# rdevooght/sequence-based-recommendations

Hardware: AMD Instinct MI355X
Metric: user-sequences/sec training (ML-1M shape, seq200 b256) at 1/2/4/8 GPUs (higher is better)
Workload: dtype f32; 1 GPU; c2: train.py -m RNN --r_t GRU --r_l 128 --max_length 200 -b 256 --loss CCE --u_m adam, N=3706 items, Zipf(1.0) ids, lengths=full, 256 rows per GPU; global_batch=256, seq_len=200, parallelism=dp1

## Files before the change

### sequence-based-recommendations_amd/csrc/sbr_api.hip

```cpp
#include "sbr_common.h"
#include <stdarg.h>
#include <stdio.h>
#include <string.h>
#include <algorithm>
#include <stdlib.h>
#include <math.h>
#include <array>
#include <atomic>
#include <chrono>

static thread_local std::string g_err;
void sbr_set_error(const char* fmt, ...) {
    char buf[1024];
    va_list ap; va_start(ap, fmt); vsnprintf(buf, sizeof(buf), fmt, ap); va_end(ap);
    g_err = buf;
}
extern "C" const char* sbr_last_error(void) { return g_err.c_str(); }
extern "C" int sbr_abi_version(void) { return SBR_ABI_VERSION; }


int sbr_build_layout(const sbr_config& cfg, Layout& lay, std::string& err) {
    char buf[256];
#define LFAIL(...) do { snprintf(buf, sizeof(buf), __VA_ARGS__); err = buf; return SBR_EINVAL; } while (0)
    if (cfg.abi_version != SBR_ABI_VERSION) LFAIL("abi_version %d != %d", cfg.abi_version, SBR_ABI_VERSION);
// ... 739 lines not shown
}

__global__ void __launch_bounds__(256) occupy_kernel(unsigned long long ticks, int* sink) {
    extern __shared__ int occ_lds[];
    occ_lds[threadIdx.x] = (int)threadIdx.x;
    const unsigned long long t0 = wall_clock64();
    while (wall_clock64() - t0 < ticks) __builtin_amdgcn_s_sleep(64);
    if (occ_lds[(threadIdx.x + 1) & 255] == -7) *sink = 1;
}
extern "C" int sbr_debug_occupy(sbr_handle* h, int workgroups, int lds_kb, int milliseconds) {
    CHECK_ARG(h && workgroups >= 0 && workgroups <= 4096 && lds_kb >= 0 && lds_kb <= 160 && milliseconds >= 0 && milliseconds <= 10000, "bad argument");
    static hipStream_t occ = nullptr;
    if (!occ) SBR_HIP(hipStreamCreateWithFlags(&occ, hipStreamNonBlocking));
    if (workgroups == 0) { SBR_HIP(hipStreamSynchronize(occ)); return SBR_OK; }
    const size_t lds = std::max<size_t>(1024, (size_t)lds_kb * 1024);
    SBR_DYN_LDS(occupy_kernel, lds);
    occupy_kernel<<<workgroups, 256, lds, occ>>>((unsigned long long)milliseconds * 100000ull, (int*)h->A(h->lay.a_fault) + 1);
    SBR_LAUNCH(hipGetLastError());
    return SBR_OK;
}

extern "C" int sbr_query(sbr_handle* h, const char* what, int64_t* value) {
    CHECK_ARG(h && what && value, "null argument");
    const Layout& y = h->lay; const std::string w(what);
    const RecPlan& top = h->plan[(y.L - 1) * y.D];
    if (w == "fused_gather") *value = h->plan[0].fuse_gather ? 1 : 0;
    else if (w == "rows_per_workgroup") *value = h->rpt;
    else if (w == "head_fused") {
        int cc = 0, cw = 0; size_t lds = 0;
        *value = (h->sw.head_fuse && y.cfg.loss == SBR_LOSS_CCE && !simple_gemm(h) && !(y.cfg.flags & (SBR_FLAG_BF16_PROJECTION | SBR_FLAG_F32_MFMA)) &&
                  y.D == 1 && y.B == y.Bp && sbr_head_plan(y.Bp, y.N, y.HLt, &cc, &cw, &lds) && (size_t)cc * y.Bp * y.HLt <= y.ws_floats) ? cc : 0;
    }
    else if (w == "head_sampled") *value = head_sampled_taken(h, y.B) ? 1 : 0;
    else if (w == "scatter_form") *value = h->last_scatter_form;
    else if (w == "step_join_gate") *value = h->last_join_gate;
    else if (w == "step_fork_gate") *value = h->last_fork_gate;
    else if (w == "tail_gate_first") *value = h->last_tail_gated;
    else if (w == "rank_select") *value = h->last_rank_select;
    else if (w == "rank_sort") *value = h->last_rank_sort;
    else if (w == "cluster_rank_form") *value = h->last_cluster_rank_form;
    else if (w == "goal_rank_form") *value = h->last_goal_rank_form;
    else if (w == "goal_rank_tile") *value = kGoalRankTile;
    else if (w == "row_aware_update") *value = h->last_row_aware ? 1 : 0;
    else if (w == "cluster") *value = top.needs_fill ? 1 : 0;
    else if (w == "rec_kernel") *value = top.family;
    else if (w.rfind("rec_products_", 0) == 0 || w.rfind("rec_rows_", 0) == 0 || w.rfind("rec_workgroups_", 0) == 0) {
        const bool bwd = w.size() > 4 && w.compare(w.size() - 4, 4, "_bwd") == 0;
        *value = w.rfind("rec_products_", 0) == 0 ? (bwd ? top.products_bwd : top.products_fwd)
               : w.rfind("rec_rows_", 0) == 0 ? (bwd ? top.bwd_rows : top.fwd_rows) : (bwd ? top.bwd_wgs : top.fwd_wgs);
    }
    else if (w == "tail_chunks") *value = h->tail_chunks;
    else if (w == "tail_streams") *value = (h->tail_chunks >= 2 && h->sw.tail_overlap == 1) ? 1 : 0;
    else if (w == "tail_last_steps") *value = h->tail_chunks >= 2 ? h->tail_bounds.lo[1] : 0;
    else if (w == "side_stream2") *value = (int64_t)(intptr_t)h->side2;
    else if (w == "tail_chain_cycles" || w == "tail_chain_ticks") {
        unsigned long long c[2] = {0, 0};
        const int nwaves = (y.Bp / h->rpt) * 8;
        SBR_HIP(hipStreamSynchronize(h->stream));
        SBR_HIP(hipMemcpy(c, (const int*)h->A(y.a_prog) + nwaves + 128, sizeof(c), hipMemcpyDeviceToHost));
        *value = (int64_t)c[w == "tail_chain_cycles" ? 0 : 1];
    }
    else if (w == "tail_win_lo") *value = (int64_t)y.layer[0].p_Win;
    else if (w == "tail_win_hi") *value = (int64_t)y.layer[0].p_b;
    else if (w == "tail_whid_lo") *value = (int64_t)y.layer[0].p_Whid;
    else if (w == "tail_whid_hi") *value = (int64_t)y.layer[0].p_peep;
    else if (w == "arena_bytes") *value = (int64_t)(y.s_end * sizeof(float));
    else if (w == "sparse_blocks") *value = y.n_sparse;
    else if (w == "adam_table") *value = y.n_at;
    else if (w == "side_stream") *value = (int64_t)(intptr_t)h->side;
    else { sbr_set_error("unknown query '%s'", what); return SBR_EINVAL; }
    return SBR_OK;
}

extern "C" int sbr_enable_timing(sbr_handle* h, int on) {
    CHECK_ARG(h, "null handle");
    if (on)
        for (int r = 0; r < sbr_handle::kRing; ++r)
            for (int i = 0; i < SBR_N_PHASES; ++i) if (!h->ev[r][i]) SBR_HIP(hipEventCreate(&h->ev[r][i]));
    CHECK_ARG(on >= 0 && on <= SBR_N_PHASES, "on = %d: 0 off, 1 every phase, 2 + p only phase p", on);
    h->timing = on != 0; h->ring_used = 0; h->ring_cur = 0;
    h->timing_marks = on == 1 ? 0xffu : on >= 2 ? (3u << (on - 2)) : 0u;
    return SBR_OK;
}

extern "C" int sbr_chain_times(sbr_handle* h, int on, float us[2], int n[2]) {
    CHECK_ARG(h, "null handle");
    if (on) { h->ch_n = 0; h->chain_timing = true; return SBR_OK; }
    CHECK_ARG(us && n, "null argument");
    h->chain_timing = false;
    SBR_HIP(hipDeviceSynchronize());
    us[0] = us[1] = 0.f; n[0] = n[1] = 0;
    for (int r = 0; r < h->ch_n; ++r) {
        float ms = 0.f;
        if (!h->ev_ch[r][0] || !h->ev_ch[r][1] || hipEventElapsedTime(&ms, h->ev_ch[r][0], h->ev_ch[r][1]) != hipSuccess) continue;
        us[h->ch_dir[r] & 1] += ms * 1000.f; n[h->ch_dir[r] & 1] += 1;
    }
    h->ch_n = 0;
    return SBR_OK;
}

extern "C" int sbr_phase_times(sbr_handle* h, float us[SBR_N_PHASES]) {
    CHECK_ARG(h && us, "null argument");
    if (!h->timing || h->ring_used == 0) { sbr_set_error("no timed train step recorded"); return SBR_ESTATE; }
    SBR_HIP(hipStreamSynchronize(h->stream));
    const int n = std::min(h->ring_used, (int)sbr_handle::kRing);
    for (int i = 0; i < SBR_N_PHASES; ++i) us[i] = 0.f;
// ... 11 lines not shown
```

### sequence-based-recommendations_amd/csrc/sbr_common.h

```cpp
#pragma once
#include <hip/hip_runtime.h>
#include <stdint.h>
#include <stddef.h>
#include <math.h>
#include <string>
#include <vector>
#include "../../include/sbr_rnn.h"
#include "sbr_upd.h"

#define SBR_BWD_CHUNKS 4
#define SBR_ALIGN_FLOATS 64

static inline size_t sbr_align(size_t n_floats) { return (n_floats + SBR_ALIGN_FLOATS - 1) / SBR_ALIGN_FLOATS * SBR_ALIGN_FLOATS; }
static inline int sbr_gates(int cell) { return cell == SBR_CELL_LSTM ? 4 : (cell == SBR_CELL_GRU ? 3 : 1); }
static inline int sbr_pad_hidden(int H) {
    if (H <= 16) return 16;
    if (H <= 32) return 32;
    if (H <= 64) return 64;
    if (H <= 128) return 128;
    if (H <= 256) return 256;
    if (H <= 512) return 512;
    return (H + 63) / 64 * 64;
}

// ... 50 lines not shown
    size_t a_dhl[2];
    size_t a_dinp[2];
    size_t a_s2cnt, a_s2off, a_s2cur, a_s2sid, a_s2pos;
    int E, Ep;
    size_t p_Emb;
    size_t a_emb, a_demb;
    LayerLayout layer[2 * SBR_MAX_LAYERS];
    size_t p_WoutT, p_bout;
    size_t n_params;
    size_t p_split;
    size_t n_state_arrays;
    size_t s_params, s_grads, s_state, s_act, s_end;
    size_t a_logits;
    size_t a_dhlast;
    size_t a_rowcost;
    int NT;
    size_t a_dflt;
    size_t a_Wc, a_bc, a_act, a_dWc, a_dbc;
    size_t a_ws; size_t ws_floats;
    size_t a_ws2; size_t ws2_floats;
    size_t a_csum;
    size_t a_prof;
    size_t a_fault;
    size_t a_clx;
    size_t a_X, a_len, a_tgt, a_smp, a_cells, a_pop, a_topk;
    size_t a_X2, a_len2, a_tgt2, a_smp2, a_pop2;
    size_t a_scnt, a_soff, a_scur, a_sid, a_spos;
    size_t a_sP;
    size_t a_hstat;
    size_t a_srpart, a_srid; int sr_slots;
    int tail_keys;
    size_t a_prog;
    size_t a_done;
};

int sbr_build_layout(const sbr_config& cfg, Layout& lay, std::string& err);

struct ParamDesc { std::string name; int layer; int kind; int gate; int64_t d0, d1; int ndim; };
void sbr_param_descs(const Layout& lay, std::vector<ParamDesc>& out);

#define SBR_TCHUNKS_MAX 9
struct SbrTChunks { int n; int lo[SBR_TCHUNKS_MAX + 1]; };
constexpr int kWgradSlices = 256;
constexpr int kWgradX6Wgs = 512;
constexpr int kTailChunksMax = 8;
constexpr int kTailPubEvery = 2;
constexpr int kTailShortChunks = 3;
constexpr int kTailFenceKb = 124;
constexpr int kTailFirst = 6;
constexpr int kTailScatterUnits = 192;
constexpr int kTailGemmGroups = 64;
constexpr int kTailSlabMax = 512;
constexpr double kTailSlabGrowth = 0.35;
constexpr bool kTailGateFirst = true;
constexpr int kTailGateSleep = 32;
constexpr bool kStepJoinGate = true;
constexpr bool kStepForkGate = true;
static inline double sbr_tail_geom(int scatter_lds) { return scatter_lds ? 1.6 : 2.6; }

enum ScatForm { SCAT_REDUCE = 0, SCAT_RANGE = 1, SCAT_WIDE = 2, SCAT_ATOMIC = 3, SCAT_POLL = 4, SCAT_LDS = 5 };
struct ScatReduce { int nv; bool comb; };
struct ScatPlan {
    ScatForm plain = SCAT_REDUCE, tail = SCAT_POLL;
    ScatReduce reduce = {0, false};
    int range_nv = 0, wide_nvw = 0, wide_nvb = 0;
    int poll_nv = 0;
    int lds_nv = 0, floor_cost = 0, rows_lds = 0;
    bool wide_rows = false;
};
static inline bool sbr_scatter_wide_rows(int Ep, int GHp) { return !Ep && GHp >= 512 && GHp <= 8192; }
static inline int sbr_scatter_wide_slots(size_t max_entries) { return (int)(max_entries / 64 + max_entries / 65 + 2); }
ScatReduce sbr_scat_reduce_recipe(int row_floats);
ScatPlan sbr_scat_plan(int GHp, int Ep, int n_ids, int entries, int D, bool atomic, int scat_range, int tail_scatter_lds,
                       int tail_chunks, int units, int part_slots);
constexpr int kRankThreads = 1024;
constexpr int kRankLdsRow = 32768;
constexpr int kRankSortLds = 2048;
constexpr int kGoalRankTile = 1024;
static_assert(kGoalRankTile == kRankThreads, "ev_goal_rank_kernel: a thread owns one goal item of the tile and one word of its scan");

__device__ __forceinline__ unsigned rank_key(float v) {
    if (!(v > -INFINITY)) return 0u;
    unsigned u = __float_as_uint(v);
    if (v == 0.0f) u = 0u;
    return (u & 0x80000000u) ? ~u : (u | 0x80000000u);
}

struct UserSplit {
    int L, half, fed;
    __host__ __device__ constexpr UserSplit(long long off_lo, long long off_hi, int T)
        : L((int)(off_hi - off_lo)), half(L / 2), fed(T < half ? T : half) {}
    __host__ __device__ constexpr int goal_len() const { return L - half; }
    __host__ __device__ constexpr int viewed_begin() const { return 0; }
    __host__ __device__ constexpr int viewed_end() const { return half; }
    __host__ __device__ constexpr int window_begin() const { return half - fed; }
    __host__ __device__ constexpr int window_end() const { return half; }
};
#define SBR_SPLIT_IS(L, T, H, G, WB) (UserSplit(100, 100 + (L), (T)).half == (H) && UserSplit(100, 100 + (L), (T)).goal_len() == (G) && \
                                      UserSplit(100, 100 + (L), (T)).window_begin() == (WB) && UserSplit(100, 100 + (L), (T)).window_end() == (H))
static_assert(SBR_SPLIT_IS(2, 0, 1, 1, 1) && SBR_SPLIT_IS(2, 1, 1, 1, 0) && SBR_SPLIT_IS(2, 5, 1, 1, 0), "L = 2: one item viewed, one the goal");
static_assert(SBR_SPLIT_IS(3, 0, 1, 2, 1) && SBR_SPLIT_IS(3, 1, 1, 2, 0) && SBR_SPLIT_IS(3, 2, 1, 2, 0), "L = 3: the odd item belongs to the goal");
static_assert(SBR_SPLIT_IS(7, 2, 3, 4, 1) && SBR_SPLIT_IS(7, 3, 3, 4, 0) && SBR_SPLIT_IS(7, 4, 3, 4, 0), "L = 7: the window is the END of the viewed half");
#undef SBR_SPLIT_IS

#define HEAD_WAIT_TICKS 6000ull
struct SbrSwitches {
// ... 168 lines not shown
void plan_tail(sbr_handle* h);
bool head_sampled_taken(const sbr_handle* h, int rows);
void mark(sbr_handle* h, int i);
SbrSparseRows sparse_rows(sbr_handle* h, int b);
SbrSparseUpd sparse_upd(sbr_handle* h);
int side_join(sbr_handle* h);
static inline bool sparse_lazy(const sbr_handle* h) { return h->lay.n_sparse > 0 && h->lay.cfg.updater != SBR_UPD_ADAGRAD; }
struct SbrSortKeys { int *cnt, *off, *cur, *sid, *pos; };
SbrSortKeys sort_keys(const sbr_handle* h, int dir);
std::vector<std::pair<size_t, size_t>> sparse_float_ranges(const Layout& lay);

#define SBR_DYN_LDS(KERNEL, LDS) do { static int sbr_dyn_lds_set_ = -1; if ((int)(LDS) > sbr_dyn_lds_set_) { \
        (void)hipFuncSetAttribute((const void*)KERNEL, hipFuncAttributeMaxDynamicSharedMemorySize, (int)(LDS)); sbr_dyn_lds_set_ = (int)(LDS); } } while (0)
#define SBR_DONE_COPIES 32
#define SBR_DONE_STRIDE 1088
struct SbrPoll { const int* words; int n; int* done; int epoch; int rows_per_step; int* fault; int n_small, k_small;
                 unsigned long long* trace; const int* slab_lo; int n_slabs; };

hipError_t launch_gather_xt(hipStream_t s, const float* Win, const float* bias, const int* X, float* xt,
                            int T, int Bp, int F, int GHp, int n_rows_in);
hipError_t launch_scatter_rows(hipStream_t s, float* dWin, const float* dxt, const int* X, const int* len,
                               int T, int Bp, int F, int GHp);
hipError_t launch_scatter_sort(hipStream_t s, const int* X, const int* len, int T, int Bp, int F, int n_ids, int* cnt,
                               int* offs, int* cur, int* sid, int* spos, int concat = 0, int tch = 0, int n_tchunks = 1, const SbrTChunks* bounds = nullptr,
                               int* cnt_zero_n = nullptr);
int sbr_scatter_lds_ids();
hipError_t launch_tail_gate(hipStream_t s, const int* progress, int n, int epoch, int target, int* fault);
hipError_t launch_tail_gate_wave(hipStream_t s, const int* progress, int n, int epoch, int target, int* fault);
hipError_t launch_step_gate(hipStream_t s, const int* w0, const int* w1, int epoch, int* fault);
hipError_t launch_step_word(hipStream_t s, int* word, int epoch);
hipError_t launch_gather_concat(hipStream_t s, const float* Wemb, const int* X, float* out, int T, int Bp, int F, int Ep);
hipError_t launch_rev_rows_int(hipStream_t s, const int* X, const int* len, int* Xr, int T, int Bp, int F);
hipError_t launch_rev_rows(hipStream_t s, const float* src, const int* len, float* dst, int T, int Bp, int W);
hipError_t launch_cat_outputs(hipStream_t s, const float* hs_f, const float* hs_b, const int* len, float* cat, int T, int Bp, int Hp);
hipError_t launch_hcat(hipStream_t s, const float* hf, const float* hb, float* out, int Bp, int Hp);
hipError_t launch_split_cols(hipStream_t s, const float* src, float* a, float* b, int rows, int Hp);
hipError_t launch_uncat(hipStream_t s, const float* f, const float* r, const int* len, float* out_f, float* out_b, int T, int Bp,
                        int W, int Hp);
hipError_t launch_scatter_range(hipStream_t s, float* dWin, const float* dxt, const int* sid, const int* spos, const int* offs, int n_ids,
                                int GHp, float* part, int* part_id, int n_ranges, const ScatPlan& plan);
#define SBR_SCAT_RANGES 512
hipError_t launch_scatter_wide(hipStream_t s, float* dWin, const float* dxt, const int* sid, const int* spos, const int* offs, int n_ids,
                               int max_entries, int GHp, float* part, int* aux, int n_slots, const ScatPlan& plan);
hipError_t launch_scatter_reduce(hipStream_t s, float* dWin, const float* dxt, const int* sid, const int* spos,
                                 const int* offs, int n_ids, int max_entries, int GHp, int Bp, const ScatReduce& recipe);
hipError_t launch_scatter_reduce_poll(hipStream_t s, float* dWin, const float* dxt, const int* sid, const int* spos, const int* offs,
                                      int n_ids, int n_tchunks, int max_entries, int GHp, int Bp, const SbrPoll& poll,
                                      const SbrTChunks& bounds, int short_chunks, bool fence_on, const ScatPlan& plan);
hipError_t launch_scatter_cost_scan(hipStream_t s, const int* offs, int* P, int n_ids, int n_tchunks, const ScatPlan& plan);
hipError_t launch_scatter_lds_poll(hipStream_t s, float* dWin, const float* dxt, const int* sid, const int* spos, const int* offs, const int* P,
                                   int n_ids, int n_tchunks, int GHp, const SbrPoll& poll, const SbrTChunks& bounds,
                                   int units, const ScatPlan& plan, bool monitor = false, int t_lo = 0);
hipError_t launch_tail_monitor(hipStream_t s, const SbrPoll& poll, int t_lo);

__host__ __device__ __forceinline__ size_t sbr_blocked_index(int t, int row, int col, int Bp, int ncols) {
    return (((size_t)t * (Bp >> 4) + (row >> 4)) * (ncols >> 4) + (col >> 4)) * 256 + (row & 15) * 16 + (col & 15);
}

struct RecArgs {
    int cell, T, Bp, H, Hp, G;
    float clip;
    const int* len;
    const float* xt;
    const float* Whid;
    const float* peep;
    const float* cinit;
    const float* hinit;
    float* hs; float* cs; float* g[4];
    const float* dh_last;
    const float* dh_slabs;
    int n_dh_slabs;
    const float* dh_ext;
    int dhe_on;
    float* dxt; float* dhi;
    int t_lo, t_hi, chunk;
    float* state;
    float* part;
    int rpt;
    int xt_blocked;
    int x6_pipe;
    int x6_f16, x6_f16_bwd;
    int cl16, c16_two_level;
    const int* gX;
    const float* gWin;
    int n_in;
    const float* gbias;
    int f32_mfma;
    unsigned long long* prof;
    int cluster;
    int cl_linear;
    int* fault;
    int sentinel_done;
    int* clx;
    void* xh;
    float* pring;
    int epoch;
    int relu;
    int* progress; int prog_every; int prog_epoch;
    int* start_word; int start_epoch;
    int fence_kb;
};
static inline bool sbr_rec_f16_fwd(const RecArgs& a) { return a.x6_f16 && !a.relu; }
static inline bool sbr_rec_f16_bwd(const RecArgs& a) { return a.x6_f16_bwd && a.clip > 0.0f && a.clip <= 100.0f; }
#define SBR_CL_ROWS 8
#define SBR_C16_RING 2
#define SBR_X6P_FUSE_MAX_T 4096
// ... 128 lines not shown
```

### sequence-based-recommendations_amd/csrc/sbr_misc.hip

```cpp
#include "sbr_common.h"
#include "sbr_rec_p.h"
#include "sbr_device.h"
#include <math.h>

typedef float f32x4 __attribute__((ext_vector_type(4)));


__global__ void gather_xt_kernel(const f32x4* __restrict__ Win, const f32x4* __restrict__ bias,
                                 const int* __restrict__ X, f32x4* __restrict__ xt, int T, int Bp, int F, int R4) {
    const size_t total = (size_t)T * Bp * R4;
    for (size_t i = (size_t)blockIdx.x * blockDim.x + threadIdx.x; i < total; i += (size_t)gridDim.x * blockDim.x) {
        const int f4 = (int)(i % R4);
        const size_t pos = i / R4;
        const int b = (int)(pos % Bp), t = (int)(pos / Bp);
        f32x4 v = bias[f4];
        const int* ids = X + ((size_t)b * T + t) * F;
        for (int f = 0; f < F; ++f) v += Win[(size_t)ids[f] * R4 + f4];
        xt[i] = v;
    }
}

__global__ void gather_concat_kernel(const f32x4* __restrict__ W, const int* __restrict__ X, f32x4* __restrict__ out, int T,
                                     int Bp, int F, int E4) {
    const size_t total = (size_t)T * Bp * F * E4;
// ... 76 lines not shown
    const int w = i % (2 * Hp), r = i / (2 * Hp);
    if (w < Hp) a[(size_t)r * Hp + w] = src[i]; else b[(size_t)r * Hp + w - Hp] = src[i];
}
hipError_t launch_split_cols(hipStream_t s, const float* src, float* a, float* b, int rows, int Hp) {
    split_cols_kernel<<<(rows * 2 * Hp + 255) / 256, 256, 0, s>>>(src, a, b, rows, Hp);
    return hipGetLastError();
}

__global__ void uncat_kernel(const float* __restrict__ f, const float* __restrict__ r, const int* __restrict__ len,
                             float* __restrict__ out_f, float* __restrict__ out_b, int T, int Bp, int W, int Hp) {
    const size_t total = (size_t)T * Bp * W;
    for (size_t i = (size_t)blockIdx.x * blockDim.x + threadIdx.x; i < total; i += (size_t)gridDim.x * blockDim.x) {
        const int w = (int)(i % W);
        const size_t pos = i / W;
        const int b = (int)(pos % Bp), t = (int)(pos / Bp);
        const int tr = rev_t(t, len[b]);
        const float d = f[i] + r[((size_t)tr * Bp + b) * W + w];
        if (!out_b) out_f[i] = d;
        else if (w < Hp) out_f[((size_t)t * Bp + b) * Hp + w] = d;
        else out_b[((size_t)tr * Bp + b) * Hp + (w - Hp)] = d;
    }
}
hipError_t launch_uncat(hipStream_t s, const float* f, const float* r, const int* len, float* out_f, float* out_b, int T, int Bp,
                        int W, int Hp) {
    const size_t total = (size_t)T * Bp * W;
    uncat_kernel<<<(int)min((size_t)4096, (total + 255) / 256), 256, 0, s>>>(f, r, len, out_f, out_b, T, Bp, W, Hp);
    return hipGetLastError();
}

hipError_t launch_gather_xt(hipStream_t s, const float* Win, const float* bias, const int* X, float* xt, int T, int Bp,
                            int F, int GHp, int) {
    const int R4 = GHp / 4;
    const size_t total = (size_t)T * Bp * R4;
    const int grid = (int)min((size_t)256 * 16, (total + 255) / 256);
    gather_xt_kernel<<<grid, 256, 0, s>>>((const f32x4*)Win, (const f32x4*)bias, X, (f32x4*)xt, T, Bp, F, R4);
    return hipGetLastError();
}

__global__ void __launch_bounds__(512) tail_gate_kernel(const int* __restrict__ progress, int n, int epoch, int target, int* __restrict__ fault) {
    for (int i = threadIdx.x; i < n; i += blockDim.x) {
        const unsigned long long t0 = wall_clock64();
        for (;;) {
            const int v = __hip_atomic_load(progress + i, __ATOMIC_RELAXED, __HIP_MEMORY_SCOPE_AGENT);
            if ((v >> 12) == epoch && (v & 0xfff) <= target) break;
            if (wall_clock64() - t0 > SBR_POLL_TICKS) { atomicOr(fault, 8); break; }
            __builtin_amdgcn_s_sleep(8);
        }
    }
}

__global__ void __launch_bounds__(256) tail_monitor_kernel(SbrPoll pl, int t_lo) { tail_monitor_loop(pl, t_lo); }
hipError_t launch_tail_monitor(hipStream_t s, const SbrPoll& poll, int t_lo) {
    tail_monitor_kernel<<<1, 256, 0, s>>>(poll, t_lo);
    return hipGetLastError();
}

hipError_t launch_tail_gate(hipStream_t s, const int* progress, int n, int epoch, int target, int* fault) {
    tail_gate_kernel<<<1, 512, 0, s>>>(progress, n, epoch, target, fault);
    return hipGetLastError();
}

__global__ void __launch_bounds__(64) tail_gate_wave_kernel(const int* __restrict__ progress, int n, int epoch, int target, int* __restrict__ fault) {
    const unsigned long long t0 = wall_clock64();
    auto passed = [&](int v) { return (v >> 12) == epoch && (v & 0xfff) <= target; };
    for (;;) {
        if (passed(__hip_atomic_load(progress, __ATOMIC_RELAXED, __HIP_MEMORY_SCOPE_AGENT))) break;
        if (wall_clock64() - t0 > SBR_POLL_TICKS) { if (threadIdx.x == 0) atomicOr(fault, 8); return; }
        __builtin_amdgcn_s_sleep(kTailGateSleep);
    }
    for (;;) {
        bool ok = true;
#pragma unroll 8
        for (int i = 0; i < n; i += 64)
            ok = passed(__hip_atomic_load(progress + min(i + (int)threadIdx.x, n - 1), __ATOMIC_RELAXED, __HIP_MEMORY_SCOPE_AGENT)) && ok;
        if (__all(ok)) break;
        if (wall_clock64() - t0 > SBR_POLL_TICKS) { if (threadIdx.x == 0) atomicOr(fault, 8); return; }
        __builtin_amdgcn_s_sleep(8);
    }
}
hipError_t launch_tail_gate_wave(hipStream_t s, const int* progress, int n, int epoch, int target, int* fault) {
    if (n < 1) return hipErrorInvalidValue;
    tail_gate_wave_kernel<<<1, 64, 0, s>>>(progress, n, epoch, target, fault);
    return hipGetLastError();
}

__global__ void __launch_bounds__(64) step_gate_kernel(const int* __restrict__ w0, const int* __restrict__ w1, int epoch, int* __restrict__ fault) {
    const unsigned long long t0 = wall_clock64();
    for (;;) {
        const int a = __hip_atomic_load(w0, __ATOMIC_RELAXED, __HIP_MEMORY_SCOPE_AGENT);
        const int b = w1 ? __hip_atomic_load(w1, __ATOMIC_RELAXED, __HIP_MEMORY_SCOPE_AGENT) : epoch;
        if (a == epoch && b == epoch) break;
        if (wall_clock64() - t0 > SBR_POLL_TICKS) { if (threadIdx.x == 0) atomicOr(fault, 8); return; }
        __builtin_amdgcn_s_sleep(8);
    }
}
hipError_t launch_step_gate(hipStream_t s, const int* w0, const int* w1, int epoch, int* fault) {
    if (!w0 || !epoch) return hipErrorInvalidValue;
    step_gate_kernel<<<1, 64, 0, s>>>(w0, w1, epoch, fault);
    return hipGetLastError();
}
__global__ void __launch_bounds__(64) step_word_kernel(int* __restrict__ word, int epoch) {
    if (threadIdx.x == 0) __hip_atomic_store(word, epoch, __ATOMIC_RELAXED, __HIP_MEMORY_SCOPE_AGENT);
}
hipError_t launch_step_word(hipStream_t s, int* word, int epoch) {
    if (!word || !epoch) return hipErrorInvalidValue;
    step_word_kernel<<<1, 64, 0, s>>>(word, epoch);
// ... 335 lines not shown
```

### sequence-based-recommendations_amd/csrc/sbr_scatter.hip

```cpp
#include "sbr_common.h"
#include "sbr_rec_p.h"

#define SCAT_LDS_IDS 36864
#define SCAT_BLOCK 1024
__device__ __forceinline__ int scat_key(int id, int t, const SbrTChunks& tc, int ids_per_chunk) {
    if (tc.n <= 1) return id;
    int c = 0;
#pragma unroll
    for (int k = 1; k < SBR_TCHUNKS_MAX; ++k) c += (k < tc.n && t >= tc.lo[k]) ? 1 : 0;
    return c * ids_per_chunk + id;
}

__global__ void __launch_bounds__(SCAT_BLOCK) scat_count_lds_kernel(const int* __restrict__ X, const int* __restrict__ len,
                                                                    int T, int Bp, int F, int n_ids, int per_block,
                                                                    int* __restrict__ cnt, SbrTChunks tch, int ipc) {
    extern __shared__ int hist[];
    for (int i = threadIdx.x; i < n_ids; i += SCAT_BLOCK) hist[i] = 0;
    __syncthreads();
    const int total = T * Bp * F;
    const int lo = blockIdx.x * per_block, hi = min(total, lo + per_block);
    for (int i = lo + threadIdx.x; i < hi; i += SCAT_BLOCK) {
        const int f = i % F, pos = i / F, b = pos % Bp, t = pos / Bp;
        if (t < len[b]) atomicAdd(&hist[scat_key(X[((size_t)b * T + t) * F + f], t, tch, ipc)], 1);
    }
// ... 166 lines not shown
        const int f = i % F; pos = i / F;
        const int b = pos % Bp, t = pos / Bp;
        if (t < len[b]) { id = X[((size_t)b * T + t) * F + f]; h = scat_agg_insert(hkey, hcnt, id, rank); }
    }
    __syncthreads();
    for (int k = threadIdx.x; k < SCAT_AGG_SLOTS; k += 1024) if (hkey[k] >= 0) hbase[k] = atomicAdd(&cur[hkey[k]], hcnt[k]);
    __syncthreads();
    if (id >= 0) { const int slot = hbase[h] + rank; sid[slot] = id; spos[slot] = concat ? i : pos; }
}

int sbr_scatter_lds_ids() { return SCAT_LDS_IDS; }

hipError_t launch_scatter_sort(hipStream_t s, const int* X, const int* len, int T, int Bp, int F, int n_ids, int* cnt,
                               int* offs, int* cur, int* sid, int* spos, int concat, int tch, int n_tchunks, const SbrTChunks* bounds,
                               int* cnt_zero_n) {
    const int ipc = n_ids;
    const SbrTChunks tc = bounds ? *bounds : SbrTChunks{};
    if (tch > 0) {
        n_ids *= n_tchunks;
        if (n_ids > SCAT_LDS_IDS || tc.n != n_tchunks || tc.n > SBR_TCHUNKS_MAX || tc.lo[0] != 0 || tc.lo[tc.n] < T) return hipErrorInvalidValue;
    }
    if (!(cnt_zero_n && *cnt_zero_n >= n_ids)) {
        hipError_t e = hipMemsetAsync(cnt, 0, (size_t)n_ids * sizeof(int), s);
        if (e != hipSuccess) return e;
    }
    if (cnt_zero_n) *cnt_zero_n = n_ids <= SCAT_LDS_IDS ? n_ids : 0;
    const int total = T * Bp * F;
    if (n_ids <= SCAT_LDS_IDS) {
        const int per_block = 4096;
        const int grid = (total + per_block - 1) / per_block;
        const size_t lds = (size_t)n_ids * sizeof(int);
        SBR_DYN_LDS(scat_count_lds_kernel, lds);
        SBR_DYN_LDS(scat_fill_lds_kernel, lds);
        scat_count_lds_kernel<<<grid, SCAT_BLOCK, lds, s>>>(X, len, T, Bp, F, n_ids, per_block, cnt, tc, ipc);
        SBR_DYN_LDS(scat_scan_kernel<true>, lds);
        scat_scan_kernel<true><<<1, 1024, lds, s>>>(cnt, n_ids, offs, cur);
        scat_fill_lds_kernel<<<grid, SCAT_BLOCK, lds, s>>>(X, len, T, Bp, F, n_ids, per_block, cur, sid, spos, concat, tc, ipc);
    } else {
        const int agrid = (total + 1023) / 1024;
        scat_count_agg_kernel<<<agrid, 1024, 0, s>>>(X, len, T, Bp, F, cnt);
        const int nb = (n_ids + SCAN_BLK - 1) / SCAN_BLK;
        if (nb <= 1) scat_scan_kernel<false><<<1, 1024, 0, s>>>(cnt, n_ids, offs, cur);
        else {
            scat_scan_local_kernel<<<nb, 1024, 0, s>>>(cnt, n_ids, offs, cur);
            scat_scan_totals_kernel<<<1, 1024, 0, s>>>(cur, nb, cnt, offs + n_ids);
            scat_scan_add_kernel<<<nb, 1024, 0, s>>>(cnt, n_ids, offs, cur);
        }
        scat_fill_agg_kernel<<<agrid, 1024, 0, s>>>(X, len, T, Bp, F, cur, sid, spos, concat);
    }
    return hipGetLastError();
}

#define SCAT_FLY 8
template <int NV, int SCAT_CHUNK, bool ACC = false, bool POLL = false>
__global__ void __launch_bounds__(256) scat_reduce_kernel(const f32x4* __restrict__ dxt, const int* __restrict__ sid,
                                                          const int* __restrict__ spos, const int* __restrict__ offs,
                                                          int n_ids, float* __restrict__ dWin, int R4, int Bp, int key_lo = 0,
                                                          int n_tchunks = 1, SbrTChunks tch = SbrTChunks(), SbrPoll poll = SbrPoll()) {
    constexpr int FLY = (NV == 1 && !POLL) ? 16 : SCAT_FLY;
    const int lane = threadIdx.x & 63;
    const int wave_global = blockIdx.x * (blockDim.x >> 6) + (threadIdx.x >> 6), n_waves = gridDim.x * (blockDim.x >> 6);
    const int total = offs[POLL ? n_ids * n_tchunks : key_lo + n_ids];
    const int e_lo = POLL ? offs[key_lo] : 0;
    constexpr int SCAT_SHORT = 8;
    const int e_mid = POLL ? max(e_lo, min(total, offs[min(poll.n_small, n_tchunks) * n_ids])) : 0;
    const int nchA = POLL ? (total - e_mid + SCAT_CHUNK - 1) / SCAT_CHUNK : 0, nchB = POLL ? (e_mid - e_lo + SCAT_SHORT - 1) / SCAT_SHORT : 0;
    for (int it = wave_global; ; it += n_waves) {
    int base, cnt;
    if (POLL) {
        if (it >= nchA + nchB) break;
        if (it < nchA) { base = e_mid + (nchA - 1 - it) * SCAT_CHUNK; cnt = min(SCAT_CHUNK, total - base); }
        else { base = e_lo + (nchB - 1 - (it - nchA)) * SCAT_SHORT; cnt = min(SCAT_SHORT, e_mid - base); }
    } else {
        base = offs[key_lo] + wave_global * SCAT_CHUNK;
        if (base >= total) return;
        cnt = min(SCAT_CHUNK, total - base);
    }
    const int lim = base + cnt;
    const int e = base + (lane & (SCAT_CHUNK - 1));
    const int my_id = e < lim ? sid[e] : -1;
    const int my_pos = e < lim ? spos[e] : 0;
    if (POLL) {
        const int t_need = tch.lo[min(__shfl(my_id, 0) / n_ids, SBR_TCHUNKS_MAX)];
        if (lane == 0) {
            const unsigned long long t0 = wall_clock64();
            const int* mine = poll.done + ((blockIdx.x + 16) & (SBR_DONE_COPIES - 1)) * SBR_DONE_STRIDE;
            for (;;) {
                const int v = __hip_atomic_load(mine, __ATOMIC_RELAXED, __HIP_MEMORY_SCOPE_AGENT);
                if ((v >> 12) == poll.epoch && (v & 0xfff) <= t_need) break;
                if (wall_clock64() - t0 > SBR_POLL_TICKS) { atomicOr(poll.fault, 8); break; }
                poll_sleep((v >> 12) == poll.epoch ? (v & 0xfff) - t_need : 64);
            }
        }
        __builtin_amdgcn_wave_barrier();
        if (poll.trace && lane == 0) {
            const int k = min((it - wave_global) / n_waves, 3);
            poll.trace[8192 + (wave_global * 4 + k) * 2] = wall_clock64();
        }
    }
    f32x4 acc[NV];
#pragma unroll
    for (int v = 0; v < NV; ++v) acc[v] = f32x4{0, 0, 0, 0};
    int cur_id = __shfl(my_id, 0);
#ifndef SCAT_DEBUG_NOFLUSH
#define SCAT_DEBUG_NOFLUSH 0
#endif
// ... 654 lines not shown
```

### sequence-based-recommendations_amd/csrc/sbr_step.hip

```cpp
#include "sbr_common.h"
#include <string.h>
#include <algorithm>
#include <atomic>
#include <chrono>

static inline unsigned long long* prof_slot(const sbr_handle* h, int k) {
    return (unsigned long long*)h->A(h->lay.a_prof) + (size_t)k * (h->lay.Bp / 16) * 16 * 8;
}
static RecArgs rec_shape(const sbr_handle* h, int l) {
    const Layout& y = h->lay; const LayerLayout& ly = y.layer[l];
    RecArgs a; memset(&a, 0, sizeof(a));
    a.cell = y.cfg.cell; a.T = y.T; a.Bp = y.Bp; a.H = ly.H; a.Hp = ly.Hp; a.G = y.G;
    a.n_in = ly.n_in_p;
    a.clip = y.cfg.grad_clip;
    a.rpt = h->rpt; a.x6_pipe = h->sw.x6_pipe; a.x6_f16 = h->sw.x6_f16; a.x6_f16_bwd = h->sw.x6_f16_bwd;
    a.cl16 = h->sw.cl16; a.c16_two_level = h->sw.c16_two_level;
    a.hs = h->A(ly.a_hs); a.cs = h->A(ly.a_cs);
    for (int k = 0; k < 4; ++k) a.g[k] = h->A(ly.a_g[k]);
    if (ly.Hp == 256 || ly.Hp == 512) { a.xh = h->A(ly.a_xh); a.pring = h->A(ly.a_pring); }
    a.f32_mfma = (y.cfg.flags & SBR_FLAG_F32_MFMA) ? 1 : 0;
    a.prof = (y.cfg.flags & SBR_FLAG_PROFILE_REC) ? prof_slot(h, 0) : nullptr;
    a.cluster = h->sw.cluster; a.cl_linear = h->sw.cl_linear;
    a.relu = (y.cfg.cell == SBR_CELL_VANILLA && (l / y.D > 0 || y.E)) ? 1 : 0;
    return a;
// ... 1 lines not shown
static RecArgs rec_args(sbr_handle* h, int l) {
    const Layout& y = h->lay; const LayerLayout& ly = y.layer[l];
    RecArgs a = rec_shape(h, l);
    a.len = h->blen;
    a.xt = h->A(ly.a_xt); a.Whid = h->P(ly.p_Whid); a.peep = h->P(ly.p_peep);
    a.cinit = h->P(ly.p_cinit); a.hinit = h->P(ly.p_hinit);
    a.dxt = h->A(ly.a_dxt); a.dhi = h->A(ly.a_dhi); a.part = h->A(ly.a_part);
    a.xt_blocked = 0;
    a.t_lo = 0; a.t_hi = y.T; a.chunk = 0; a.state = h->A(ly.a_state);
    a.fault = (int*)h->A(y.a_fault);
    a.clx = (int*)h->A(y.a_clx); a.epoch = (++h->cl_epoch) & 0x07FFFFFF;
    return a;
}
static bool simple_rec(const sbr_handle* h) { return h->lay.cfg.flags & SBR_FLAG_SIMPLE_REC; }
void plan_layers(sbr_handle* h) {
    const Layout& y = h->lay;
    for (int l = 0; l < y.L * y.D; ++l) {
        RecArgs a = rec_shape(h, l);
        if (l / y.D < y.L - 1) a.dh_ext = h->A(y.layer[l].a_dhext);
        h->plan[l] = sbr_rec_plan(a, simple_rec(h), l / y.D == 0 && !y.E && y.F == 1 && h->sw.fuse_gather);
    }
}
static const RecPlan& plan_of(const sbr_handle* h, const LayerLayout& ly) { return h->plan[&ly - h->lay.layer]; }
static inline bool layer_gemm_f16(const sbr_handle* h, bool with_gradient) {
    const Layout& y = h->lay;
    if (!h->sw.gemm_f16 || y.cfg.cell == SBR_CELL_VANILLA) return false;
    return !with_gradient || (y.cfg.grad_clip > 0.0f && y.cfg.grad_clip <= 100.0f);
}
static inline void layer_gemm_hint(const sbr_handle* h, bool grad_a, bool grad_b) {
    if (h->lay.cfg.flags & SBR_FLAG_BF16_LAYERS) sbr_gemm_hint(1, 1.0f, 1.0f);
    else if (layer_gemm_f16(h, grad_a || grad_b)) sbr_gemm_hint(2, grad_a ? 512.0f : 1.0f, grad_b ? 512.0f : 1.0f);
}
bool simple_gemm(const sbr_handle* h) { return h->lay.cfg.flags & SBR_FLAG_SIMPLE_GEMM; }
bool head_sampled_taken(const sbr_handle* h, int rows) {
    const Layout& y = h->lay;
    return h->sw.head_fuse && !simple_gemm(h) && y.D == 1 && !(y.cfg.flags & SBR_FLAG_F32_MFMA) &&
           sbr_head_sampled_ok(rows, y.C, y.HLt, y.cfg.loss);
}
void plan_tail(sbr_handle* h) {
    const Layout& y = h->lay;
    h->tail_chunks = h->tail_ch = 0;
    if (!h->sw.tail_overlap || y.tail_keys < 2 || y.n_sparse || h->sw.bwd_chunks != 1) return;
    if (!h->plan[0].tail_ok || simple_gemm(h) || (y.cfg.flags & SBR_FLAG_ATOMIC_SCATTER)) return;
    int nc = std::min(std::min(y.tail_keys, kTailChunksMax), y.T / 16);
    if (nc < 2) return;
    const int ch = (y.T + nc - 1) / nc;
    nc = (y.T + ch - 1) / ch;
    if (nc < 2) return;
    h->tail_chunks = nc; h->tail_ch = ch;
    const double geom = sbr_tail_geom(h->sw.tail_scatter_lds);
    SbrTChunks& tc = h->tail_bounds;
    tc.n = nc;
    tc.lo[0] = 0;
    double pw = h->sw.tail_scatter_lds ? (double)kTailFirst : 1.0;
    for (int c = 0; c < nc; ++c) {
        const int rem = y.T - tc.lo[c], left = nc - c;
        const int share = (rem + left - 1) / left;
        const int n_small = nc >= 4 ? nc / 2 : (nc - 1) / 2;
        int sz = (geom > 1.0 && c < n_small) ? std::min(share, std::max(1, (int)(pw + 0.5))) : (geom > 1.0 ? share : std::min(rem, ch));
        if (c == nc - 1) sz = rem;
        sz = std::max(1, std::min(sz, rem - (left - 1)));
        tc.lo[c + 1] = tc.lo[c] + sz;
        pw *= geom > 1.0 ? geom : 1.0;
    }
    for (int c = nc; c <= SBR_TCHUNKS_MAX; ++c) tc.lo[c] = y.T;
}

static int tail_next_epoch(sbr_handle* h) {
    h->prog_epoch = (h->prog_epoch + 1) & 0x7FFFF; if (!h->prog_epoch) h->prog_epoch = 1;
    return h->prog_epoch;
}
static int step_next_epoch(int* e) { *e = (*e + 1) & 0x7FFFFFFF; if (!*e) *e = 1; return *e; }
static bool step_boundary_marks(const sbr_handle* h) { return h->timing && (h->timing_marks & ((1u << 0) | (1u << 6))); }
static int* tail_words(sbr_handle* h, int* nwaves) {
    *nwaves = (h->lay.Bp / h->rpt) * 8;
    return (int*)h->A(h->lay.a_prog);
}

SbrSortKeys sort_keys(const sbr_handle* h, int dir) {
    const Layout& y = h->lay;
    if (dir) return {(int*)h->A(y.a_s2cnt), (int*)h->A(y.a_s2off), (int*)h->A(y.a_s2cur), (int*)h->A(y.a_s2sid), (int*)h->A(y.a_s2pos)};
    return {(int*)h->A(y.a_scnt), (int*)h->A(y.a_soff), (int*)h->A(y.a_scur), (int*)h->A(y.a_sid), (int*)h->A(y.a_spos)};
}
static inline int sort_entries(const Layout& y) { return y.T * y.Bp * y.F; }

static int tail_sort(sbr_handle* h) {
    const Layout& y = h->lay; const SbrSortKeys k = sort_keys(h, 0);
    SBR_LAUNCH(launch_scatter_sort(h->side2, h->bX, h->blen, y.T, y.Bp, y.F, y.cfg.input_size, k.cnt, k.off, k.cur, k.sid, k.pos, 0,
                                   h->tail_ch, h->tail_nc, &h->tail_bounds, &h->scnt_zero_n));
    if (h->scat.tail == SCAT_LDS)
        SBR_LAUNCH(launch_scatter_cost_scan(h->side2, k.off, (int*)h->A(y.a_sP), y.cfg.input_size, h->tail_nc, h->scat));
    return SBR_OK;
}

static inline void chain_mark(sbr_handle* h, hipStream_t st, int dir, int which) {
    if (!h->chain_timing || h->ch_n >= sbr_handle::kChain) return;
    hipEvent_t& e = h->ev_ch[h->ch_n][which];
    if (!e && hipEventCreate(&e) != hipSuccess) { e = nullptr; return; }
    (void)hipEventRecord(e, st);
    if (which == 1) { h->ch_dir[h->ch_n] = (unsigned char)dir; h->ch_n += 1; }
}
#define SBR_LAUNCH_CHAIN(DIR, STREAM, CALL) do { chain_mark(h, STREAM, DIR, 0); SBR_LAUNCH(CALL); chain_mark(h, STREAM, DIR, 1); } while (0)

static inline bool mark_live(const sbr_handle* h, int i) { return h->timing && ((h->timing_marks >> i) & 1) && h->ev[h->ring_cur][i]; }
static inline void mark_on(sbr_handle* h, int i, hipStream_t st) {
    if (i == 0) h->marks_shared = 0;
    if ((h->marks_shared >> i) & 1) return;
    if (mark_live(h, i)) (void)hipEventRecord(h->ev[h->ring_cur][i], st);
}
void mark(sbr_handle* h, int i) { mark_on(h, i, h->stream); }
static inline hipEvent_t record_shared(sbr_handle* h, hipEvent_t plain, int mk) {
    if (mk >= 0 && mark_live(h, mk)) {
// ... 499 lines not shown
    p.f16 = h->sw.wgrad_f16 && !a.relu && y.cfg.grad_clip > 0.0f && y.cfg.grad_clip <= 100.0f;
    if (p.gemm && p.nsl > 1) {
        p.nsl = std::max(1, std::min(p.nsl, kWgradX6Wgs / (((ly.Hp + 127) / 128) * ((GHp + 127) / 128)) / p.nc));
    }
    p.swap = p.side && p.nc == 1 && y.L == 1 && !y.E && !y.n_sparse &&
             y.n_params <= ((size_t)4 << 20) &&
             !(y.cfg.flags & SBR_FLAG_ATOMIC_SCATTER);
    return p;
}

static int tail_slab_table(sbr_handle* h, int K, int cap, SbrPoll* pl) {
    if (h->tail_slab_key[0] != K || h->tail_slab_key[1] != cap || !h->tail_slab_dev) {
        sbr_tail_slab_table(K, h->lay.Bp, 255, kTailSlabGrowth, kTailSlabMax, h->tail_slab_host);
        if (!h->tail_slab_dev) SBR_HIP(hipMalloc(&h->tail_slab_dev, 260 * sizeof(int)));
        SBR_HIP(hipMemcpy(h->tail_slab_dev, h->tail_slab_host.data(), h->tail_slab_host.size() * sizeof(int), hipMemcpyHostToDevice));
        h->tail_slab_key[0] = K; h->tail_slab_key[1] = cap;
    }
    pl->slab_lo = h->tail_slab_dev;
    pl->n_slabs = (int)h->tail_slab_host.size() - 1;
    return SBR_OK;
}

static int backward_tail(sbr_handle* h, RecArgs& a, const WgradPlan& wp, int nblk) {
    const Layout& y = h->lay; const LayerLayout& ly = y.layer[0];
    hipStream_t s = h->stream, sd = h->side;
    const int GHp = y.G * ly.Hp;
    const size_t slab = wp.slab;
    float* ws2 = h->A(y.a_ws2);
    const int tnc = h->tail_nc;
    const bool serial = h->sw.tail_overlap == 2;
    hipStream_t s2 = serial ? s : h->side2;
    if (serial) {
        sd = s;
        { const int rc = side_join(h); if (rc != SBR_OK) return rc; }
        SBR_HIP(hipEventRecord(h->ev_tail2, h->side2));
        SBR_HIP(hipStreamWaitEvent(s, h->ev_tail2, 0));
    }
    const bool gru = y.cfg.cell == SBR_CELL_GRU;
    int nwaves = 0;
    int* words = tail_words(h, &nwaves);
    int* done = (int*)h->A(y.a_done);
    const bool gated = h->tail_gated && !serial;
    h->tail_gated = false; h->last_tail_gated = gated;
    a.progress = words; a.prog_every = kTailPubEvery; a.prog_epoch = gated ? h->prog_epoch : tail_next_epoch(h);
    const int K = y.T * y.Bp;
    const int cap = (int)std::min<size_t>(256, y.ws2_floats / slab);
    SbrPoll pl{words, nwaves, done, a.prog_epoch, y.Bp, a.fault, 0, 0, h->tail_trace, nullptr, 0};
    { const int rc = tail_slab_table(h, K, cap, &pl); if (rc != SBR_OK) return rc; }
    const int n_slabs = std::max(1, std::min(std::min(kTailGemmGroups, cap), pl.n_slabs));
    const bool upd_here = h->in_train_step;
    if (!serial) a.fence_kb = kTailFenceKb;
    SBR_LAUNCH_CHAIN(1, s, launch_rec_backward(s, a, h->plan[0]));
    mark(h, 4);
    const bool out_early = upd_here && (y.cfg.loss == SBR_LOSS_CCE || SBR_LOSS_IS_MARGIN(y.cfg.loss));
    if (out_early && !h->out_stepped)
        SBR_LAUNCH(step_range(h, sd, y.p_split, y.n_params));
    const bool mon_in_units = !serial && h->scat.tail == SCAT_LDS;
    if (!mon_in_units) SBR_LAUNCH(launch_tail_monitor(serial ? s : h->side3, pl, a.t_lo));
    if (!gated) SBR_LAUNCH(launch_tail_gate(sd, words, nwaves, a.prog_epoch, y.T, a.fault));
    {
        hipError_t we = hipSuccess;
        if (!launch_gemm_slabs_x6_poll(sd, h->A(ly.a_hs), 1, ly.Hp, a.dxt, GHp, 1, ly.Hp, GHp, K, ws2, n_slabs, GHp, slab,
                                       gru ? a.dhi : nullptr, ly.Hp, gru ? 2 * ly.Hp : 0, &we, wp.f16 ? 2 : 3, 1.0f, wp.f16 ? 512.0f : 1.0f, pl)) {
            sbr_set_error("overlapped tail: the weight-gradient GEMM rejected the shape"); return SBR_EINVAL;
        }
        SBR_LAUNCH(we);
    }
    if (gated) SBR_LAUNCH(launch_tail_gate_wave(s2, words, nwaves, a.prog_epoch, y.T, a.fault));
    else if (!serial) SBR_LAUNCH(launch_tail_gate(s2, words, nwaves, a.prog_epoch, y.T, a.fault));
    const SbrSortKeys k = sort_keys(h, 0);
    h->last_scatter_form = h->scat.tail;
    if (h->scat.tail == SCAT_LDS)
        SBR_LAUNCH(launch_scatter_lds_poll(s2, h->Gd(ly.p_Win), a.dxt, k.sid, k.pos, k.off, (const int*)h->A(y.a_sP), y.cfg.input_size, tnc,
                                           GHp, pl, h->tail_bounds, kTailScatterUnits, h->scat, mon_in_units, a.t_lo));
    else
        SBR_LAUNCH(launch_scatter_reduce_poll(s2, h->Gd(ly.p_Win), a.dxt, k.sid, k.pos, k.off, y.cfg.input_size, tnc, sort_entries(y),
                                              GHp, y.Bp, pl, h->tail_bounds, kTailShortChunks, !serial && kTailFenceKb > 0, h->scat));
    const bool join_gate = kStepJoinGate && upd_here && !serial && !step_boundary_marks(h);
    if (join_gate) step_next_epoch(&h->join_epoch);
    h->last_join_gate = join_gate;
    if (upd_here) SBR_LAUNCH(step_range(h, s2, ly.p_Win, ly.p_b));
    if (join_gate) SBR_LAUNCH(launch_step_word(s2, h->step_words + 96, h->join_epoch));
    SBR_HIP(hipEventRecord(h->ev_tail2, s2));
    if (upd_here && ly.p_peep - ly.p_Whid == slab && (slab & 3) == 0) {
        SBR_LAUNCH(step_from_slabs(h, sd, ws2, n_slabs, ly.p_Whid, slab));
    } else {
        SBR_LAUNCH(launch_splitk_reduce(sd, ws2, n_slabs, ly.Hp, GHp, h->Gd(ly.p_Whid), GHp, nullptr));
        if (upd_here) SBR_LAUNCH(step_range(h, sd, ly.p_Whid, ly.p_peep));
    }
    if (join_gate) SBR_LAUNCH(launch_step_word(sd, h->step_words + 32, h->join_epoch));
    SBR_HIP(hipEventRecord(h->ev_tail, sd));
    SBR_LAUNCH(reduce_partials(h, s, ly, a, nblk));
    mark(h, 5);
    if (upd_here) {
        if (!out_early && h->og_recorded) SBR_HIP(hipStreamWaitEvent(s, h->ev_og, 0));
        SBR_LAUNCH(step_range(h, s, ly.p_b, out_early ? y.p_split : y.n_params, ly.p_Whid - ly.p_b, ly.p_peep - ly.p_Whid));
        h->tail_updated = true;
    }
    if (h->deferred_join && !h->in_train_step && !serial) {
        h->tail_join_pending = true;
        mark(h, 6);
        return SBR_OK;
    }
    if (join_gate) {
        SBR_LAUNCH(launch_step_gate(s, h->step_words + 32, h->step_words + 96, h->join_epoch, a.fault));
        h->side_pending = false;
// ... 390 lines not shown
```

Measured before the change: 906,300 user-sequences/s.

## Align tail chunk sizes to scatter rounds and publish end word after backward

Changes the time-chunk plan for the overlapped tail so that early small chunks are sized from one scatter round (32 entries across scatter units) and rounded to multiples of it, instead of starting from a fixed first size. It also launches a tiny kernel on the main stream after the recurrent backward that writes an epoch/t_lo completion word into the done slots, letting pollers see the end of the chain without waiting on per-step progress. The intent is to reduce idle polling and partial rounds in the overlapped weight-gradient scatter, at the cost of an extra launch and reliance on the done-word encoding.

```diff
diff --git a/sequence-based-recommendations_amd/csrc/sbr_api.hip b/sequence-based-recommendations_amd/csrc/sbr_api.hip
--- a/sequence-based-recommendations_amd/csrc/sbr_api.hip
+++ b/sequence-based-recommendations_amd/csrc/sbr_api.hip
@@ -815,6 +815,10 @@
     else if (w == "tail_chunks") *value = h->tail_chunks;
     else if (w == "tail_streams") *value = (h->tail_chunks >= 2 && h->sw.tail_overlap == 1) ? 1 : 0;
     else if (w == "tail_last_steps") *value = h->tail_chunks >= 2 ? h->tail_bounds.lo[1] : 0;
+    else if (w.rfind("tail_chunk_lo_", 0) == 0) {
+        const int c = atoi(w.c_str() + 14);
+        *value = (h->tail_chunks >= 2 && c >= 0 && c <= h->tail_chunks) ? h->tail_bounds.lo[c] : 0;
+    }
     else if (w == "side_stream2") *value = (int64_t)(intptr_t)h->side2;
     else if (w == "tail_chain_cycles" || w == "tail_chain_ticks") {
         unsigned long long c[2] = {0, 0};
diff --git a/sequence-based-recommendations_amd/csrc/sbr_common.h b/sequence-based-recommendations_amd/csrc/sbr_common.h
--- a/sequence-based-recommendations_amd/csrc/sbr_common.h
+++ b/sequence-based-recommendations_amd/csrc/sbr_common.h
@@ -126,6 +126,16 @@
 constexpr int kTailGemmGroups = 64;
 constexpr int kTailSlabMax = 512;
 constexpr double kTailSlabGrowth = 0.35;
+#ifndef SBR_TAIL_END_WORD
+#define SBR_TAIL_END_WORD 1
+#endif
+#ifndef SBR_TAIL_LAG_PLAN
+#define SBR_TAIL_LAG_PLAN 1
+#endif
+constexpr bool kTailEndWord = SBR_TAIL_END_WORD != 0;
+constexpr bool kTailLagPlan = SBR_TAIL_LAG_PLAN != 0;
+constexpr int kTailRoundEntries = 32;
+constexpr int kTailEndSteps = 16;
 constexpr bool kTailGateFirst = true;
 constexpr int kTailGateSleep = 32;
 constexpr bool kStepJoinGate = true;
@@ -400,6 +410,7 @@
                                    int n_ids, int n_tchunks, int GHp, const SbrPoll& poll, const SbrTChunks& bounds,
                                    int units, const ScatPlan& plan, bool monitor = false, int t_lo = 0);
 hipError_t launch_tail_monitor(hipStream_t s, const SbrPoll& poll, int t_lo);
+hipError_t launch_tail_end_word(hipStream_t s, int* done, int epoch, int t_lo);
 
 __host__ __device__ __forceinline__ size_t sbr_blocked_index(int t, int row, int col, int Bp, int ncols) {
     return (((size_t)t * (Bp >> 4) + (row >> 4)) * (ncols >> 4) + (col >> 4)) * 256 + (row & 15) * 16 + (col & 15);
diff --git a/sequence-based-recommendations_amd/csrc/sbr_misc.hip b/sequence-based-recommendations_amd/csrc/sbr_misc.hip
--- a/sequence-based-recommendations_amd/csrc/sbr_misc.hip
+++ b/sequence-based-recommendations_amd/csrc/sbr_misc.hip
@@ -152,6 +152,15 @@
 __global__ void __launch_bounds__(256) tail_monitor_kernel(SbrPoll pl, int t_lo) { tail_monitor_loop(pl, t_lo); }
 hipError_t launch_tail_monitor(hipStream_t s, const SbrPoll& poll, int t_lo) {
     tail_monitor_kernel<<<1, 256, 0, s>>>(poll, t_lo);
+    return hipGetLastError();
+}
+
+__global__ void __launch_bounds__(64) tail_end_word_kernel(int* __restrict__ done, int word) {
+    if (threadIdx.x < SBR_DONE_COPIES) __hip_atomic_store(done + threadIdx.x * SBR_DONE_STRIDE, word, __ATOMIC_RELAXED, __HIP_MEMORY_SCOPE_AGENT);
+}
+hipError_t launch_tail_end_word(hipStream_t s, int* done, int epoch, int t_lo) {
+    if (!done || epoch <= 0 || t_lo < 0 || t_lo > 0xffe) return hipErrorInvalidValue;
+    tail_end_word_kernel<<<1, 64, 0, s>>>(done, (epoch << 12) | t_lo);
     return hipGetLastError();
 }
 
diff --git a/sequence-based-recommendations_amd/csrc/sbr_scatter.hip b/sequence-based-recommendations_amd/csrc/sbr_scatter.hip
--- a/sequence-based-recommendations_amd/csrc/sbr_scatter.hip
+++ b/sequence-based-recommendations_amd/csrc/sbr_scatter.hip
@@ -242,6 +242,7 @@
 }
 
 #define SCAT_FLY 8
+static_assert(kTailRoundEntries == 4 * SCAT_FLY, "plan_tail sizes the last time chunks by one round of scat_lds_kernel's four waves");
 template <int NV, int SCAT_CHUNK, bool ACC = false, bool POLL = false>
 __global__ void __launch_bounds__(256) scat_reduce_kernel(const f32x4* __restrict__ dxt, const int* __restrict__ sid,
                                                           const int* __restrict__ spos, const int* __restrict__ offs,
diff --git a/sequence-based-recommendations_amd/csrc/sbr_step.hip b/sequence-based-recommendations_amd/csrc/sbr_step.hip
--- a/sequence-based-recommendations_amd/csrc/sbr_step.hip
+++ b/sequence-based-recommendations_amd/csrc/sbr_step.hip
@@ -77,12 +77,15 @@
     SbrTChunks& tc = h->tail_bounds;
     tc.n = nc;
     tc.lo[0] = 0;
-    double pw = h->sw.tail_scatter_lds ? (double)kTailFirst : 1.0;
+    const bool lag = kTailLagPlan && h->sw.tail_scatter_lds;
+    const int round_steps = std::max(1, (int)((long)kTailRoundEntries * kTailScatterUnits * 7 / 8 / std::max(1, y.Bp * y.F)));
+    double pw = lag ? (double)std::min(kTailEndSteps, round_steps) : (h->sw.tail_scatter_lds ? (double)kTailFirst : 1.0);
     for (int c = 0; c < nc; ++c) {
         const int rem = y.T - tc.lo[c], left = nc - c;
         const int share = (rem + left - 1) / left;
         const int n_small = nc >= 4 ? nc / 2 : (nc - 1) / 2;
         int sz = (geom > 1.0 && c < n_small) ? std::min(share, std::max(1, (int)(pw + 0.5))) : (geom > 1.0 ? share : std::min(rem, ch));
+        if (lag && geom > 1.0 && c < n_small && sz > round_steps) sz -= sz % round_steps;
         if (c == nc - 1) sz = rem;
         sz = std::max(1, std::min(sz, rem - (left - 1)));
         tc.lo[c + 1] = tc.lo[c] + sz;
@@ -688,6 +691,7 @@
     if (!serial) a.fence_kb = kTailFenceKb;
     SBR_LAUNCH_CHAIN(1, s, launch_rec_backward(s, a, h->plan[0]));
     mark(h, 4);
+    if (kTailEndWord && !serial) SBR_LAUNCH(launch_tail_end_word(s, done, a.prog_epoch, a.t_lo));
     const bool out_early = upd_here && (y.cfg.loss == SBR_LOSS_CCE || SBR_LOSS_IS_MARGIN(y.cfg.loss));
     if (out_early && !h->out_stepped)
         SBR_LAUNCH(step_range(h, sd, y.p_split, y.n_params));
```

Measured after the change: 913,100 user-sequences/s (median of 6 runs). About the same (+0.7%).
